# Gorilla-Lab-SCUT/GeoA3

Hardware: AMD Instinct MI355X
Metric: attack-iterations/sec (B=250, N=1024) (higher is better)
Workload: dtype f32; 1 GPU; configs[1]: PointNet 1024-pt, 250 instances sharded over 1 GPU(s) (250 on rank 0), full GeoA3 (CE + CD 1.0 + HD 0.1 + curvature 1.0 k=16), untargeted; instances_per_gpu=250, global_batch=250, npoint=1024, knn=16, classes=40, wide_mode=f16x2, presteps=150, parallelism=instance-sharded x1

## Files before the change

geoa3_amd/csrc/geom_slab.hip:

```cpp
#include <utility>
#include "geom_internal.h"
#include "geom_knn_self.h"
#include "profile.h"

namespace {

constexpr int SB_T = 1024;
constexpr int SB_NB = 512;
constexpr int SB_PPT = 8;
constexpr int SK_BLOCK = 256;
constexpr int SK_CHUNK = 1024;

struct alignas(128) SlabGeo {
  float lo, inv_w;
  int axis, pad;
};
constexpr int SB_PITCH = 544;

__device__ __forceinline__ int slab_bin(float v, float lo, float inv_w) {
  const int c = (int)floorf((v - lo) * inv_w);
  return c < 0 ? 0 : (c > SB_NB - 1 ? SB_NB - 1 : c);
}

__global__ __launch_bounds__(SB_T) void slab_bin_kernel(const float* __restrict__ pc, int N, float* __restrict__ sorted,
                                                        int32_t* __restrict__ sidx, int32_t* __restrict__ bstart,
                                                        SlabGeo* __restrict__ geo) {
  __shared__ float s_red[16][6];
  __shared__ int s_cnt[SB_NB], s_start[SB_NB + 1], s_wsum[16];
  const int b = blockIdx.x, tid = threadIdx.x, lane = tid & 63, wave = tid >> 6;
  const float* P = pc + (size_t)b * 3 * N;
  float px[SB_PPT], py[SB_PPT], pz[SB_PPT];
  float lo[3] = {S_INF, S_INF, S_INF}, hi[3] = {-S_INF, -S_INF, -S_INF};
#pragma unroll
  for (int p = 0; p < SB_PPT; ++p) {
    const int i = tid + p * SB_T;
    if (i < N) {
      px[p] = P[i];
      py[p] = P[N + i];
      pz[p] = P[2 * N + i];
      lo[0] = fminf(lo[0], px[p]); hi[0] = fmaxf(hi[0], px[p]);
      lo[1] = fminf(lo[1], py[p]); hi[1] = fmaxf(hi[1], py[p]);
      lo[2] = fminf(lo[2], pz[p]); hi[2] = fmaxf(hi[2], pz[p]);
    }
  }
#pragma unroll
  for (int c = 0; c < 3; ++c) {
    lo[c] = -wave_max(-lo[c]);
    hi[c] = wave_max(hi[c]);
  }
  if (lane == 0) {
#pragma unroll
    for (int c = 0; c < 3; ++c) {
      s_red[wave][c] = lo[c];
      s_red[wave][3 + c] = hi[c];
    }
  }
  if (tid < SB_NB) s_cnt[tid] = 0;
  __syncthreads();
#pragma unroll
  for (int w = 0; w < 16; ++w)
#pragma unroll
    for (int c = 0; c < 3; ++c) {
      lo[c] = fminf(lo[c], s_red[w][c]);
      hi[c] = fmaxf(hi[c], s_red[w][3 + c]);
    }
  const float ex = hi[0] - lo[0], ey = hi[1] - lo[1], ez = hi[2] - lo[2];
  const int axis = (ex >= ey && ex >= ez) ? 0 : (ey >= ez ? 1 : 2);
  const float alo = axis == 0 ? lo[0] : (axis == 1 ? lo[1] : lo[2]);
  const float ext = axis == 0 ? ex : (axis == 1 ? ey : ez);
  const float inv_w = ext > 1e-30f ? (float)SB_NB / (ext * 1.00001f) : 0.f;
  int bin[SB_PPT];
#pragma unroll
  for (int p = 0; p < SB_PPT; ++p) {
    const int i = tid + p * SB_T;
    if (i < N) {
      bin[p] = slab_bin(axis == 0 ? px[p] : (axis == 1 ? py[p] : pz[p]), alo, inv_w);
      atomicAdd(&s_cnt[bin[p]], 1);
    }
  }
  __syncthreads();
  int c = tid < SB_NB ? s_cnt[tid] : 0, incl = c;
#pragma unroll
  for (int o = 1; o < 64; o <<= 1) {
    const int v = __shfl_up(incl, o, 64);
    if (lane >= o) incl += v;
  }
  if (lane == 63) s_wsum[wave] = incl;
  __syncthreads();
  int base = 0;
#pragma unroll
  for (int w = 0; w < 16; ++w) base += (w < wave) ? s_wsum[w] : 0;
  if (tid < SB_NB) {
    s_start[tid] = base + incl - c;
    s_cnt[tid] = 0;
  }
  if (tid == SB_NB - 1) s_start[SB_NB] = base + incl;
  __syncthreads();
  float* S = sorted + (size_t)b * 3 * N;
#pragma unroll
  for (int p = 0; p < SB_PPT; ++p) {
    const int i = tid + p * SB_T;
    if (i < N) {
      const int pos = s_start[bin[p]] + atomicAdd(&s_cnt[bin[p]], 1);
      S[pos] = px[p];
      S[N + pos] = py[p];
      S[2 * N + pos] = pz[p];
      sidx[(size_t)b * N + pos] = i;
    }
  }
  for (int e = tid; e <= SB_NB; e += SB_T) bstart[(size_t)b * SB_PITCH + e] = s_start[e];
  if (tid == 0) geo[b] = SlabGeo{alo, inv_w, axis, 0};
}

typedef float slab_f2 __attribute__((ext_vector_type(2)));
__device__ __forceinline__ void slab_sqdist2(float nqx, float nqy, float nqz, float x0, float x1, float y0, float y1,
                                             float z0, float z1, float& d0, float& d1) {
#pragma clang fp contract(off)
  const slab_f2 dx = slab_f2{x0, x1} + slab_f2{nqx, nqx};
  const slab_f2 dy = slab_f2{y0, y1} + slab_f2{nqy, nqy};
  const slab_f2 dz = slab_f2{z0, z1} + slab_f2{nqz, nqz};
  const slab_f2 xx = dx * dx, yy = dy * dy, zz = dz * dz;
  const slab_f2 s = xx + yy;
  const slab_f2 d = s + zz;
  d0 = d.x;
  d1 = d.y;
}
__device__ __forceinline__ void slab_negq(float qx, float qy, float qz, float& nqx, float& nqy, float& nqz) {
  nqx = -qx;
  nqy = -qy;
  nqz = -qz;
  asm volatile("" : "+v"(nqx), "+v"(nqy), "+v"(nqz));
}

__device__ __forceinline__ bool slab_lex_less(float da, int ia, float db, int ib) {
  return (da < db) || (da == db && ia < ib);
}

template <int CAP>
__device__ __forceinline__ float slab_compact(uint16_t* cand, float* candd, int cnt, int K, int tid) {
  float kth = S_INF;
  if constexpr (CAP <= 40) {
    unsigned long long key[CAP];
    int rank[CAP];
#pragma unroll
    for (int s = 0; s < CAP; ++s) {
      const unsigned d = __float_as_uint(candd[s * SK_BLOCK + tid]);
      const unsigned i = cand[s * SK_BLOCK + tid];
      key[s] = s < cnt ? ((unsigned long long)d << 32) | i : ~0ull;
      rank[s] = CAP - 1 - s;
    }
#pragma unroll
    for (int i = 0; i < CAP; ++i)
#pragma unroll
      for (int j = i + 1; j < CAP; ++j) {
        unsigned long long m;
        asm volatile("v_cmp_lt_u64 %2, %3, %4\n\tv_subbrev_co_u32 %0, vcc, 0, %0, %2\n\t"
                     "v_addc_co_u32 %1, vcc, 0, %1, %2"
                     : "+v"(rank[i]), "+v"(rank[j]), "=&s"(m)
                     : "v"(key[i]), "v"(key[j])
                     : "vcc");
      }
#pragma unroll
    for (int s = 0; s < CAP; ++s) {
      if (rank[s] < K) {
        const float d = __uint_as_float((unsigned)(key[s] >> 32));
        candd[rank[s] * SK_BLOCK + tid] = d;
        cand[rank[s] * SK_BLOCK + tid] = (uint16_t)key[s];
        if (rank[s] == K - 1) kth = d;
      }
    }
    return kth;
  }
  for (int p = 0; p < K; ++p) {
    float bd = candd[p * SK_BLOCK + tid];
    int bidx = cand[p * SK_BLOCK + tid];
    int bs = p;
    for (int s = p + 1; s < cnt; ++s) {
      const float d = candd[s * SK_BLOCK + tid];
      const int i = cand[s * SK_BLOCK + tid];
      if (slab_lex_less(d, i, bd, bidx)) {
        bd = d;
        bidx = i;
        bs = s;
      }
    }
    if (bs != p) {
      candd[bs * SK_BLOCK + tid] = candd[p * SK_BLOCK + tid];
      cand[bs * SK_BLOCK + tid] = cand[p * SK_BLOCK + tid];
      candd[p * SK_BLOCK + tid] = bd;
      cand[p * SK_BLOCK + tid] = (uint16_t)bidx;
    }
    kth = bd;
  }
  return kth;
}

template <int CAP>
__global__ __launch_bounds__(SK_BLOCK) void knn_slab_kernel(const float* __restrict__ R, int N, int K,
                                                            const int32_t* __restrict__ prior,
                                                            const float* __restrict__ sorted,
                                                            const int32_t* __restrict__ sidx,
                                                            const int32_t* __restrict__ bstart,
                                                            const SlabGeo* __restrict__ geo, float* __restrict__ dists,
                                                            int32_t* __restrict__ idx) {
  extern __shared__ __attribute__((aligned(16))) unsigned char smem[];
  float* s_ref = reinterpret_cast<float*>(smem);
  float* s_cd = s_ref + 3 * SK_CHUNK;
  uint16_t* s_ci = reinterpret_cast<uint16_t*>(s_cd + (size_t)CAP * SK_BLOCK);
  uint16_t* s_id = s_ci + (size_t)CAP * SK_BLOCK;
  __shared__ int s_lo, s_hi;
  const int b = blockIdx.y, tid = threadIdx.x;
  const int pos = blockIdx.x * SK_BLOCK + tid;
  const bool live = pos < N;
  const float* Rb = R + (size_t)b * 3 * N;
  const float* Sb = sorted + (size_t)b * 3 * N;
  const int32_t* Ib = sidx + (size_t)b * N;
  const int32_t* bs = bstart + (size_t)b * SB_PITCH;
  const SlabGeo g = geo[b];
  const int pc = live ? pos : N - 1;
  const float qx = Sb[pc], qy = Sb[N + pc], qz = Sb[2 * N + pc];
  float nqx, nqy, nqz;
  slab_negq(qx, qy, qz, nqx, nqy, nqz);
  const int qo = Ib[pc];
  if (tid == 0) {
    s_lo = SB_NB;
    s_hi = -1;
  }
  float tau = S_INF;
  if (prior != nullptr && live) {
    const int32_t* pr = prior + ((size_t)b * N + qo) * K;
    float t = 0.f;
    bool ok = true;
    for (int m0 = 0; m0 < K; m0 += 8) {
      int j[8];
#pragma unroll
      for (int u = 0; u < 8; ++u) j[u] = m0 + u < K ? pr[m0 + u] : 0;
      float px[8], py[8], pz[8];
#pragma unroll
      for (int u = 0; u < 8; ++u) {
        ok = ok && j[u] >= 0 && j[u] < N;
        const int jc = j[u] < 0 ? 0 : (j[u] >= N ? N - 1 : j[u]);
        px[u] = Rb[jc];
        py[u] = Rb[N + jc];
        pz[u] = Rb[2 * N + jc];
      }
#pragma unroll
      for (int u = 0; u < 8; ++u)
        if (m0 + u < K) t = fmaxf(t, geoa3_sqdist(qx, qy, qz, px[u], py[u], pz[u]));
    }
    if (ok) tau = t;
  }
  if (!live) tau = -1.f;
  __syncthreads();
  if (live) {
    int blo = 0, bhi = SB_NB - 1;
    if (tau < S_INF) {
      const float qa = g.axis == 0 ? qx : (g.axis == 1 ? qy : qz);
      const float r = sqrtf(tau) * 1.00001f + 1e-30f;
      blo = slab_bin(qa - r, g.lo, g.inv_w);
      bhi = slab_bin(qa + r, g.lo, g.inv_w);
    }
    atomicMin(&s_lo, blo);
    atomicMax(&s_hi, bhi);
  }
  __syncthreads();
  int c_lo = bs[s_lo], c_hi = bs[s_hi + 1];

  static_assert(SK_BLOCK == 256, "aoff >> 10 is the count");
  unsigned char* const cdb = reinterpret_cast<unsigned char*>(s_cd);
  unsigned char* const cib = reinterpret_cast<unsigned char*>(s_ci);
  unsigned aoff = 4u * tid;
  int cnt = 0;
  for (int pass = 0; pass < 2; ++pass) {
    for (int c0 = c_lo; c0 < c_hi; c0 += SK_CHUNK) {
      const int cn = min(SK_CHUNK, c_hi - c0);
      const int cn4 = (cn + 3) & ~3;
      __syncthreads();
      for (int j = tid; j < cn4; j += SK_BLOCK) {
        const bool ok = j < cn;
        s_ref[j] = ok ? Sb[c0 + j] : __builtin_nanf("");
        s_ref[SK_CHUNK + j] = ok ? Sb[N + c0 + j] : __builtin_nanf("");
        s_ref[2 * SK_CHUNK + j] = ok ? Sb[2 * N + c0 + j] : __builtin_nanf("");
        s_id[j] = ok ? (uint16_t)Ib[c0 + j] : (uint16_t)0;
      }
      __syncthreads();
      float4 nx = *reinterpret_cast<const float4*>(&s_ref[0]);
      float4 ny = *reinterpret_cast<const float4*>(&s_ref[SK_CHUNK]);
      float4 nz = *reinterpret_cast<const float4*>(&s_ref[2 * SK_CHUNK]);
      for (int j = 0; j < cn4; j += 4) {
        const float4 rx = nx, ry = ny, rz = nz;
        const int jn = j + 4 < SK_CHUNK ? j + 4 : j;
        nx = *reinterpret_cast<const float4*>(&s_ref[jn]);
        ny = *reinterpret_cast<const float4*>(&s_ref[SK_CHUNK + jn]);
        nz = *reinterpret_cast<const float4*>(&s_ref[2 * SK_CHUNK + jn]);
        float da[4];
        slab_sqdist2(nqx, nqy, nqz, rx.x, rx.y, ry.x, ry.y, rz.x, rz.y, da[0], da[1]);
        slab_sqdist2(nqx, nqy, nqz, rx.z, rx.w, ry.z, ry.w, rz.z, rz.w, da[2], da[3]);
        const uint2 ids = *reinterpret_cast<const uint2*>(&s_id[j]);
        const unsigned id4[4] = {ids.x & 0xffffu, ids.x >> 16, ids.y & 0xffffu, ids.y >> 16};
#pragma unroll
        for (int u = 0; u < 4; ++u) {
          *reinterpret_cast<float*>(cdb + aoff) = da[u];
          *reinterpret_cast<uint16_t*>(cib + (aoff >> 1)) = (uint16_t)id4[u];
          aoff += da[u] <= tau ? 4u * SK_BLOCK : 0u;
        }
        if (__builtin_expect(__any(aoff > (unsigned)(CAP - 4) * 4u * SK_BLOCK + 4u * SK_BLOCK - 1u), 0)) {
          cnt = (int)(aoff >> 10);
          if (cnt >= K) {
            tau = slab_compact<CAP>(s_ci, s_cd, cnt, K, tid);
            aoff = (unsigned)K * 4u * SK_BLOCK + 4u * tid;
          }
        }
      }
    }
    cnt = (int)(aoff >> 10);
    const bool short_list = live && cnt < K && K <= N;
    if (!__syncthreads_or(short_list)) break;
    tau = live ? S_INF : -1.f;
    cnt = 0;
    aoff = 4u * tid;
    c_lo = 0;
    c_hi = N;
  }

  if (live) {
    const int keep = cnt < K ? cnt : K;
    slab_compact<CAP>(s_ci, s_cd, cnt, keep, tid);
    float* od = dists + ((size_t)b * N + qo) * K;
    int32_t* oi = idx + ((size_t)b * N + qo) * K;
    for (int m = 0; m < K; ++m) {
      od[m] = m < keep ? s_cd[m * SK_BLOCK + tid] : S_INF;
      oi[m] = m < keep ? (int32_t)s_ci[m * SK_BLOCK + tid] : -1;
    }
  }
}

template <typename F, int... S>
__device__ __forceinline__ void sp_static_for_impl(F&& f, std::integer_sequence<int, S...>) {
  (f(std::integral_constant<int, S>{}), ...);
}
template <int N_, typename F>
__device__ __forceinline__ void sp_static_for(F&& f) {
  sp_static_for_impl(f, std::make_integer_sequence<int, N_>{});
}
__device__ __forceinline__ void sp_count_less(int& r, unsigned long long kj, unsigned long long ki) {
  asm volatile("v_cmp_lt_u64 vcc, %1, %2\n\tv_addc_co_u32 %0, vcc, 0, %0, vcc" : "+v"(r) : "v"(kj), "v"(ki) : "vcc");
}

template <int SP_CAP, bool MULTI>
__global__ __launch_bounds__(SK_BLOCK) __attribute__((amdgpu_waves_per_eu(MULTI ? 3 : 4, MULTI ? 3 : 4))) void knn_slabp_kernel(const float* __restrict__ R, int N, int K,
                                                             const int32_t* __restrict__ prior,
                                                             const float* __restrict__ sorted,
                                                             const int32_t* __restrict__ sidx,
                                                             const int32_t* __restrict__ bstart,
                                                             const SlabGeo* __restrict__ geo, float* __restrict__ dists,
                                                             int32_t* __restrict__ idx) {
  __shared__ __attribute__((aligned(16))) float s_ref[3 * SK_CHUNK];
  __shared__ __attribute__((aligned(16))) uint16_t s_id[SK_CHUNK];
  constexpr int SP_KMAX = 20;
  constexpr int SP_SEED = 3 * SK_CHUNK * 4 + SK_BLOCK * SP_KMAX * 2;
  constexpr int SP_UNION = !MULTI && SP_SEED > SP_CAP * SK_BLOCK * 2 ? SP_SEED : SP_CAP * SK_BLOCK * 2;
  __shared__ __attribute__((aligned(16))) unsigned char s_un[SP_UNION];
  uint16_t* const s_pos = reinterpret_cast<uint16_t*>(s_un);
  __shared__ int s_lo, s_hi;
  const int b = blockIdx.y, tid = threadIdx.x;
  const int pos = blockIdx.x * SK_BLOCK + tid;
  const bool live = pos < N;
  const float* Rb = R + (size_t)b * 3 * N;
  const float* Sb = sorted + (size_t)b * 3 * N;
  const int32_t* Ib = sidx + (size_t)b * N;
  const int32_t* bs = bstart + (size_t)b * SB_PITCH;
  const SlabGeo g = geo[b];
  const int pc = live ? pos : N - 1;
  const float qx = Sb[pc], qy = Sb[N + pc], qz = Sb[2 * N + pc];
  float nqx, nqy, nqz;
  slab_negq(qx, qy, qz, nqx, nqy, nqz);
  const int qo = Ib[pc];
  if (tid == 0) {
    s_lo = SB_NB;
    s_hi = -1;
  }
  float tau = S_INF;
  if (!MULTI && prior != nullptr) {
    float* const s_org = reinterpret_cast<float*>(s_un);
    uint16_t* const s_pri = reinterpret_cast<uint16_t*>(s_un + 3 * SK_CHUNK * 4);
    for (int j = tid; j < 3 * N; j += SK_BLOCK) s_org[j] = Rb[j];
    s_id[tid] = (uint16_t)qo;
    __syncthreads();
    const int w0 = tid & ~63, lane = tid & 63;
    const float inv_k = 1.0f / (float)K;
    for (int e = lane; e < 64 * K; e += 64) {
      const int row = (int)(((float)e + 0.5f) * inv_k), m = e - row * K;
      const int32_t v = prior[((size_t)b * N + s_id[w0 + row]) * K + m];
      s_pri[w0 * K + e] = (uint16_t)(v < 0 || v >= N ? 0xffff : v);
    }
    __syncthreads();
    if (live) {
      float t = 0.f;
      bool ok = true;
      for (int m = 0; m < K; ++m) {
        const unsigned j = s_pri[tid * K + m];
        ok = ok && j != 0xffffu;
        const int jc = j >= (unsigned)N ? N - 1 : (int)j;
        t = fmaxf(t, geoa3_sqdist(qx, qy, qz, s_org[jc], s_org[N + jc], s_org[2 * N + jc]));
      }
      if (ok) tau = t;
    }
  }
  if (MULTI && prior != nullptr && live) {
    const int32_t* pr = prior + ((size_t)b * N + qo) * K;
    float t = 0.f;
    bool ok = true;
    for (int m0 = 0; m0 < K; m0 += 8) {
      int j[8];
#pragma unroll
      for (int u = 0; u < 8; ++u) j[u] = m0 + u < K ? pr[m0 + u] : 0;
      float px[8], py[8], pz[8];
#pragma unroll
      for (int u = 0; u < 8; ++u) {
        ok = ok && j[u] >= 0 && j[u] < N;
        const int jc = j[u] < 0 ? 0 : (j[u] >= N ? N - 1 : j[u]);
        px[u] = Rb[jc];
        py[u] = Rb[N + jc];
        pz[u] = Rb[2 * N + jc];
      }
#pragma unroll
      for (int u = 0; u < 8; ++u)
        if (m0 + u < K) t = fmaxf(t, geoa3_sqdist(qx, qy, qz, px[u], py[u], pz[u]));
    }
    if (ok) tau = t;
  }
  if (!live) tau = -1.f;
  __syncthreads();
  int blo = SB_NB, bhi = -1;
  if (live) {
    blo = 0;
    bhi = SB_NB - 1;
    if (tau < S_INF) {
      const float qa = g.axis == 0 ? qx : (g.axis == 1 ? qy : qz);
      const float r = sqrtf(tau) * 1.00001f + 1e-30f;
      blo = slab_bin(qa - r, g.lo, g.inv_w);
      bhi = slab_bin(qa + r, g.lo, g.inv_w);
    }
    atomicMin(&s_lo, blo);
    atomicMax(&s_hi, bhi);
  }
  const int w_blo = -(int)wave_max(-(float)blo), w_bhi = (int)wave_max((float)bhi);
  int wv_lo = w_blo <= w_bhi ? bs[w_blo] : 0, wv_hi = w_blo <= w_bhi ? bs[w_bhi + 1] : 0;
  __syncthreads();
  int c_lo = bs[s_lo], c_hi = bs[s_hi + 1];

  static_assert(SK_BLOCK == 256, "poff >> 9 is the count");
  unsigned char* const pb = reinterpret_cast<unsigned char*>(s_pos);
  unsigned poff = 2u * tid;
  unsigned long long key[SP_CAP];
  auto load_keys = [&](auto C_, int cnt) {
    sp_static_for<decltype(C_)::value>([&](auto S_) {
      constexpr int s = decltype(S_)::value;
      unsigned p = s_pos[s * SK_BLOCK + tid];
      float d;
      unsigned id;
      if (MULTI) {
        p = p < (unsigned)N ? p : 0u;
        d = geoa3_sqdist(qx, qy, qz, Sb[p], Sb[N + p], Sb[2 * N + p]);
        id = (unsigned)Ib[p];
      } else {
        p &= SK_CHUNK - 1;
        d = geoa3_sqdist(qx, qy, qz, s_ref[p], s_ref[SK_CHUNK + p], s_ref[2 * SK_CHUNK + p]);
        id = s_id[p];
      }
      key[s] = s < cnt ? ((unsigned long long)__float_as_uint(d) << 32) | (id << 16) | p : ~0ull;
      if ((s & 7) == 7) __builtin_amdgcn_sched_barrier(0);
    });
  };
  auto rank_of = [&](auto C_, auto S_) {
    constexpr int s = decltype(S_)::value;
    int r = 0;
    sp_static_for<decltype(C_)::value>([&](auto J_) {
      constexpr int j = decltype(J_)::value;
      if constexpr (j != s) sp_count_less(r, key[j], key[s]);
    });
    return r;
  };
  for (int pass = 0; pass < 2; ++pass) {
   for (int c0 = c_lo; c0 < c_hi; c0 += SK_CHUNK) {
    const int cn = min(SK_CHUNK, c_hi - c0);
    const int cn4 = (cn + 3) & ~3;
    __syncthreads();
    for (int j = tid; j < cn4; j += SK_BLOCK) {
      const bool ok = j < cn;
      s_ref[j] = ok ? Sb[c0 + j] : __builtin_nanf("");
      s_ref[SK_CHUNK + j] = ok ? Sb[N + c0 + j] : __builtin_nanf("");
      s_ref[2 * SK_CHUNK + j] = ok ? Sb[2 * N + c0 + j] : __builtin_nanf("");
      s_id[j] = ok ? (uint16_t)Ib[c0 + j] : (uint16_t)0;
    }
    __syncthreads();
    const int j_lo = min(max(wv_lo - c0, 0), SK_CHUNK - 4) & ~3, j_hi = (min(wv_hi - c0, cn) + 3) & ~3;
    float4 nx = *reinterpret_cast<const float4*>(&s_ref[j_lo]);
    float4 ny = *reinterpret_cast<const float4*>(&s_ref[SK_CHUNK + j_lo]);
    float4 nz = *reinterpret_cast<const float4*>(&s_ref[2 * SK_CHUNK + j_lo]);
    for (int j = j_lo; j < j_hi; j += 4) {
      const float4 rx = nx, ry = ny, rz = nz;
      const int jn = j + 4 < SK_CHUNK ? j + 4 : j;
      nx = *reinterpret_cast<const float4*>(&s_ref[jn]);
      ny = *reinterpret_cast<const float4*>(&s_ref[SK_CHUNK + jn]);
      nz = *reinterpret_cast<const float4*>(&s_ref[2 * SK_CHUNK + jn]);
      float da[4];
      slab_sqdist2(nqx, nqy, nqz, rx.x, rx.y, ry.x, ry.y, rz.x, rz.y, da[0], da[1]);
      slab_sqdist2(nqx, nqy, nqz, rx.z, rx.w, ry.z, ry.w, rz.z, rz.w, da[2], da[3]);
#pragma unroll
      for (int u = 0; u < 4; ++u) {
        *reinterpret_cast<uint16_t*>(pb + poff) = (uint16_t)((MULTI ? c0 : 0) + j + u);
        poff += da[u] <= tau ? 2u * SK_BLOCK : 0u;
      }
      if (__builtin_expect(__any(poff > (unsigned)(SP_CAP - 4) * 2u * SK_BLOCK + 2u * SK_BLOCK - 1u), 0)) {
        const int cnt = (int)(poff >> 9);
        if (cnt >= K) {
          load_keys(std::integral_constant<int, SP_CAP>{}, cnt);
          sp_static_for<SP_CAP>([&](auto S_) {
            constexpr int s = decltype(S_)::value;
            const int r = rank_of(std::integral_constant<int, SP_CAP>{}, S_);
            if (r < K) s_pos[r * SK_BLOCK + tid] = (uint16_t)key[s];
            if (r == K - 1) tau = __uint_as_float((unsigned)(key[s] >> 32));
          });
          poff = (unsigned)K * 2u * SK_BLOCK + 2u * tid;
        }
      }
    }
   }
    const int cnt = (int)(poff >> 9);
    const bool short_list = live && cnt < K && K <= N;
    if (!__syncthreads_or(short_list)) break;
    tau = live ? S_INF : -1.f;
    poff = 2u * tid;
    c_lo = 0;
    c_hi = N;
    wv_lo = 0;
    wv_hi = N;
  }

  if constexpr (MULTI) {
    if (live) {
      const int cnt = (int)(poff >> 9);
      const int keep = cnt < K ? cnt : K;
      constexpr std::integral_constant<int, SP_CAP> C_{};
      load_keys(C_, cnt);
      float* od = dists + ((size_t)b * N + qo) * K;
      int32_t* oi = idx + ((size_t)b * N + qo) * K;
      sp_static_for<SP_CAP>([&](auto S_) {
        constexpr int s = decltype(S_)::value;
        const int r = rank_of(C_, S_);
        if (r < keep) {
          od[r] = __uint_as_float((unsigned)(key[s] >> 32));
          oi[r] = (int32_t)((key[s] >> 16) & 0xffffu);
        }
      });
      for (int m = keep; m < K; ++m) {
        od[m] = S_INF;
        oi[m] = -1;
      }
    }
  } else {
    const int cnt = live ? (int)(poff >> 9) : 0;
    const int keep = cnt < K ? cnt : K;
    const int cls = !__any(cnt > 20) ? 0 : (!__any(cnt > 28) ? 1 : 2);
    constexpr std::integral_constant<int, 20> C20{};
    constexpr std::integral_constant<int, 28> C28{};
    constexpr std::integral_constant<int, SP_CAP> CXX{};
    if (cls == 0) load_keys(C20, cnt);
    else if (cls == 1) load_keys(C28, cnt);
    else load_keys(CXX, cnt);
    __syncthreads();
    float* const s_od = reinterpret_cast<float*>(s_un);
    uint16_t* const s_oi = reinterpret_cast<uint16_t*>(s_ref);
    s_id[tid] = (uint16_t)qo;
    for (int m = keep; m < K; ++m) {
      s_od[tid * K + m] = S_INF;
      s_oi[tid * K + m] = 0xffff;
    }
    auto rank_out = [&](auto C_) {
      sp_static_for<decltype(C_)::value>([&](auto S_) {
        constexpr int s = decltype(S_)::value;
        const int r = rank_of(C_, S_);
        if (r < keep) {
          s_od[tid * K + r] = __uint_as_float((unsigned)(key[s] >> 32));
          s_oi[tid * K + r] = (uint16_t)(key[s] >> 16);
        }
      });
    };
    if (cls == 0) rank_out(C20);
    else if (cls == 1) rank_out(C28);
    else rank_out(CXX);
    __syncthreads();
    const float inv_k = 1.0f / (float)K;
    const int rows = min(SK_BLOCK, N - (int)blockIdx.x * SK_BLOCK);
    for (int e = tid; e < rows * K; e += SK_BLOCK) {
      const int row = (int)(((float)e + 0.5f) * inv_k), m = e - row * K;
      const size_t o = ((size_t)b * N + s_id[row]) * K + m;
      const unsigned v = s_oi[e];
      dists[o] = s_od[e];
      idx[o] = v == 0xffffu ? -1 : (int32_t)v;
    }
  }
}

enum KnnRoute {
  ALLPAIRS = GEOA3_KNN_ROUTE_ALLPAIRS,
  CELLGRID = GEOA3_KNN_ROUTE_CELLGRID,
  SLAB40 = GEOA3_KNN_ROUTE_SLAB40,
  SLAB72 = GEOA3_KNN_ROUTE_SLAB72,
  SLAB96 = GEOA3_KNN_ROUTE_SLAB96,
  SLABP32 = GEOA3_KNN_ROUTE_SLABP32,
  SLABP56 = GEOA3_KNN_ROUTE_SLABP56,
};
constexpr int KNN_SORT_MAX_N = SB_T * SB_PPT;
constexpr int KNN_SHORT_K = 20;
constexpr int KNN_MID_K = 40;
constexpr int KNN_GRID_MIN_N = 2048;
constexpr size_t KNN_DENSE_MIN_WGS = 512;
static_assert(KNN_SORT_MAX_N <= 65535, "positions and original indices travel as 16 bits");

bool knn_self_sizes_ok(int B, int N, int K) { return B > 0 && N > 0 && K > 0 && K <= GEOA3_KNN_MAX_K; }

KnnRoute knn_self_route(int B, int N, int K, int method, bool has_prior, bool scratch_ok) {
  if (!has_prior || !scratch_ok || N > KNN_SORT_MAX_N || K > N) return ALLPAIRS;
  if (method == GEOA3_KNN_SELF_GRID || (method == GEOA3_KNN_SELF_AUTO && (K > KNN_SHORT_K || N >= KNN_GRID_MIN_N)))
    return CELLGRID;
  const size_t wgs = (size_t)((N + SK_BLOCK - 1) / SK_BLOCK) * B;
  const bool positions =
      method != GEOA3_KNN_SELF_SLAB_LISTS && (wgs > KNN_DENSE_MIN_WGS || method == GEOA3_KNN_SELF_SLAB_POSITIONS);
  if (K <= KNN_SHORT_K && N <= SK_CHUNK && positions) return SLABP32;
  if (K <= KNN_MID_K && positions) return SLABP56;
  return K <= KNN_SHORT_K ? SLAB40 : (K <= KNN_MID_K ? SLAB72 : SLAB96);
}

template <int CAP, class Launch>
void launch_slab(Launch&& launch) {
  const size_t lds = 3 * SK_CHUNK * 4 + (size_t)CAP * SK_BLOCK * 6 + SK_CHUNK * 2;
  if (lds > 64 * 1024)
    (void)hipFuncSetAttribute(reinterpret_cast<const void*>(knn_slab_kernel<CAP>), hipFuncAttributeMaxDynamicSharedMemorySize,
                              (int)lds);
  launch(knn_slab_kernel<CAP>, lds);
}

}

extern "C" int64_t geoa3_knn_self_scratch_bytes(int B, int N) {
  if (B <= 0 || N <= 0) return -1;
  const size_t a = knn_self_carve(nullptr, B, N, SB_PITCH, sizeof(SlabGeo)).total, g = geoa3_knn_cellgrid_scratch_bytes(B, N);
  return (int64_t)(a > g ? a : g);
}

extern "C" int geoa3_debug_knn_self_route(int B, int N, int K, int method, int has_prior, int scratch_ok) {
  if (!knn_self_sizes_ok(B, N, K)) return GEOA3_EINVAL;
  return knn_self_route(B, N, K, method, has_prior != 0, scratch_ok != 0);
}

extern "C" int geoa3_knn_self(const float* pc, int B, int N, int K, const int32_t* prior, float* dists, int32_t* idx,
                              void* scratch, int method, void* stream) {
  if (!pc || !dists || !idx || !knn_self_sizes_ok(B, N, K)) return GEOA3_EINVAL;
  hipStream_t s = geoa3_stream(stream);
  geoa3_prof_begin(GEOA3_PROF_KNN, s);
  int rc = GEOA3_OK;
  const bool scratch_ok = scratch && ((uintptr_t)scratch & 255) == 0;
  auto slab = [&](auto kernel, size_t lds) {
    const KnnSelfScratch sc = knn_self_carve(scratch, B, N, SB_PITCH, sizeof(SlabGeo));
    SlabGeo* const geo = static_cast<SlabGeo*>(sc.geo);
    hipLaunchKernelGGL(slab_bin_kernel, dim3(B), dim3(SB_T), 0, s, pc, N, sc.sorted, sc.sidx, sc.start, geo);
    hipLaunchKernelGGL(kernel, dim3((N + SK_BLOCK - 1) / SK_BLOCK, B), dim3(SK_BLOCK), lds, s, pc, N, K, prior, sc.sorted,
                       sc.sidx, sc.start, geo, dists, idx);
    if (hipGetLastError() != hipSuccess) rc = GEOA3_ELAUNCH;
  };
  switch (knn_self_route(B, N, K, method, prior != nullptr, scratch_ok)) {
    case ALLPAIRS: rc = geoa3_launch_knn(pc, pc, B, N, N, K, prior, dists, idx, nullptr, s); break;
    case CELLGRID: rc = geoa3_launch_knn_cellgrid(pc, B, N, K, prior, dists, idx, scratch, s); break;
    case SLAB40: launch_slab<40>(slab); break;
    case SLAB72: launch_slab<72>(slab); break;
    case SLAB96: launch_slab<96>(slab); break;
    case SLABP32: slab(knn_slabp_kernel<32, false>, 0); break;
    case SLABP56: slab(knn_slabp_kernel<56, true>, 0); break;
  }
  geoa3_prof_end(GEOA3_PROF_KNN, s);
  return rc;
}
```

Baseline: 651.8 iterations/s of a 250-instance batch.

## Prefetch slab reference chunk into registers and overlap with prior-gather setup

```diff
diff --git a/geoa3_amd/csrc/geom_slab.hip b/geoa3_amd/csrc/geom_slab.hip
--- a/geoa3_amd/csrc/geom_slab.hip
+++ b/geoa3_amd/csrc/geom_slab.hip
@@ -194,6 +194,37 @@
   }
   return kth;
 }
+
+struct SlabRun {
+  static constexpr int T = SK_CHUNK / SK_BLOCK;
+  float x[T], y[T], z[T];
+  int32_t id[T];
+  __device__ __forceinline__ void request(const float* __restrict__ Sb, const int32_t* __restrict__ Ib, int N, int c0, int cn,
+                                          int tid) {
+#pragma unroll
+    for (int u = 0; u < T; ++u) {
+      const int j = c0 + max(min(tid + u * SK_BLOCK, cn - 1), 0);
+      x[u] = Sb[j];
+      y[u] = Sb[N + j];
+      z[u] = Sb[2 * N + j];
+      id[u] = Ib[j];
+    }
+  }
+  __device__ __forceinline__ void commit(float* s_ref, uint16_t* s_id, int cn, int tid) const {
+    const int cn4 = (cn + 3) & ~3;
+#pragma unroll
+    for (int u = 0; u < T; ++u) {
+      const int j = tid + u * SK_BLOCK;
+      if (j < cn4) {
+        const bool ok = j < cn;
+        s_ref[j] = ok ? x[u] : __builtin_nanf("");
+        s_ref[SK_CHUNK + j] = ok ? y[u] : __builtin_nanf("");
+        s_ref[2 * SK_CHUNK + j] = ok ? z[u] : __builtin_nanf("");
+        s_id[j] = ok ? (uint16_t)id[u] : (uint16_t)0;
+      }
+    }
+  }
+};
 
 template <int CAP>
 __global__ __launch_bounds__(SK_BLOCK) void knn_slab_kernel(const float* __restrict__ R, int N, int K,
@@ -275,14 +306,10 @@
     for (int c0 = c_lo; c0 < c_hi; c0 += SK_CHUNK) {
       const int cn = min(SK_CHUNK, c_hi - c0);
       const int cn4 = (cn + 3) & ~3;
+      SlabRun run;
+      run.request(Sb, Ib, N, c0, cn, tid);
       __syncthreads();
-      for (int j = tid; j < cn4; j += SK_BLOCK) {
-        const bool ok = j < cn;
-        s_ref[j] = ok ? Sb[c0 + j] : __builtin_nanf("");
-        s_ref[SK_CHUNK + j] = ok ? Sb[N + c0 + j] : __builtin_nanf("");
-        s_ref[2 * SK_CHUNK + j] = ok ? Sb[2 * N + c0 + j] : __builtin_nanf("");
-        s_id[j] = ok ? (uint16_t)Ib[c0 + j] : (uint16_t)0;
-      }
+      run.commit(s_ref, s_id, cn, tid);
       __syncthreads();
       float4 nx = *reinterpret_cast<const float4*>(&s_ref[0]);
       float4 ny = *reinterpret_cast<const float4*>(&s_ref[SK_CHUNK]);
@@ -346,6 +373,23 @@
 __device__ __forceinline__ void sp_count_less(int& r, unsigned long long kj, unsigned long long ki) {
   asm volatile("v_cmp_lt_u64 vcc, %1, %2\n\tv_addc_co_u32 %0, vcc, 0, %0, vcc" : "+v"(r) : "v"(kj), "v"(ki) : "vcc");
 }
+
+#ifdef GEOA3_SP_STAMPS
+__device__ unsigned long long g_sp_stamps[8 * 16];
+#define SP_STAMP(i)                                                                                                    \
+  do {                                                                                                                 \
+    if (!MULTI && tid == 0 && blockIdx.x == 1 && (blockIdx.y & 31) == 7 && blockIdx.y < 256)                           \
+      g_sp_stamps[(blockIdx.y >> 5) * 16 + (i)] = __builtin_amdgcn_s_memtime();                                        \
+  } while (0)
+#define SP_STAMP_AFTER(i, v)                                                                                           \
+  do {                                                                                                                 \
+    asm volatile("" ::"v"(v));                                                                                         \
+    SP_STAMP(i);                                                                                                       \
+  } while (0)
+#else
+#define SP_STAMP(i)
+#define SP_STAMP_AFTER(i, v)
+#endif
 
 template <int SP_CAP, bool MULTI>
 __global__ __launch_bounds__(SK_BLOCK) __attribute__((amdgpu_waves_per_eu(MULTI ? 3 : 4, MULTI ? 3 : 4))) void knn_slabp_kernel(const float* __restrict__ R, int N, int K,
@@ -372,11 +416,13 @@
   const int32_t* bs = bstart + (size_t)b * SB_PITCH;
   const SlabGeo g = geo[b];
   const int pc = live ? pos : N - 1;
+  const int qo = Ib[pc];
   const float qx = Sb[pc], qy = Sb[N + pc], qz = Sb[2 * N + pc];
-  float nqx, nqy, nqz;
-  slab_negq(qx, qy, qz, nqx, nqy, nqz);
-  const int qo = Ib[pc];
-  if (tid == 0) {
+  SP_STAMP(0);
+  constexpr bool EARLY = !MULTI;
+  SlabRun run;
+  if (EARLY && prior == nullptr) run.request(Sb, Ib, N, 0, N, tid);
+  if (!EARLY && tid == 0) {
     s_lo = SB_NB;
     s_hi = -1;
   }
@@ -384,16 +430,33 @@
   if (!MULTI && prior != nullptr) {
     float* const s_org = reinterpret_cast<float*>(s_un);
     uint16_t* const s_pri = reinterpret_cast<uint16_t*>(s_un + 3 * SK_CHUNK * 4);
-    for (int j = tid; j < 3 * N; j += SK_BLOCK) s_org[j] = Rb[j];
-    s_id[tid] = (uint16_t)qo;
-    __syncthreads();
+    constexpr int CT = 3 * SK_CHUNK / SK_BLOCK;
+    const int n3 = 3 * N;
+    float cl[CT];
+#pragma unroll
+    for (int u = 0; u < CT; ++u) cl[u] = Rb[min(tid + u * SK_BLOCK, n3 - 1)];
     const int w0 = tid & ~63, lane = tid & 63;
     const float inv_k = 1.0f / (float)K;
-    for (int e = lane; e < 64 * K; e += 64) {
+    int32_t pv[SP_KMAX];
+    SP_STAMP_AFTER(1, qo);
+#pragma unroll
+    for (int u = 0; u < SP_KMAX; ++u) {
+      const int e = min(lane + 64 * u, 64 * K - 1);
       const int row = (int)(((float)e + 0.5f) * inv_k), m = e - row * K;
-      const int32_t v = prior[((size_t)b * N + s_id[w0 + row]) * K + m];
-      s_pri[w0 * K + e] = (uint16_t)(v < 0 || v >= N ? 0xffff : v);
-    }
+      pv[u] = prior[((size_t)b * N + __shfl(qo, row, 64)) * K + m];
+    }
+    if constexpr (EARLY) run.request(Sb, Ib, N, 0, N, tid);
+#pragma unroll
+    for (int u = 0; u < CT; ++u) s_org[tid + u * SK_BLOCK] = cl[u];
+    SP_STAMP(2);
+#pragma unroll
+    for (int u = 0; u < SP_KMAX; ++u) asm volatile("" : "+v"(pv[u]));
+#pragma unroll
+    for (int u = 0; u < SP_KMAX; ++u) {
+      const int e = lane + 64 * u;
+      if (e < 64 * K) s_pri[w0 * K + e] = (uint16_t)(pv[u] < 0 || pv[u] >= N ? 0xffff : pv[u]);
+    }
+    SP_STAMP(3);
     __syncthreads();
     if (live) {
       float t = 0.f;
@@ -431,7 +494,10 @@
     if (ok) tau = t;
   }
   if (!live) tau = -1.f;
-  __syncthreads();
+  SP_STAMP(4);
+  float nqx, nqy, nqz;
+  slab_negq(qx, qy, qz, nqx, nqy, nqz);
+  if (!EARLY) __syncthreads();
   int blo = SB_NB, bhi = -1;
   if (live) {
     blo = 0;
@@ -442,13 +508,22 @@
       blo = slab_bin(qa - r, g.lo, g.inv_w);
       bhi = slab_bin(qa + r, g.lo, g.inv_w);
     }
-    atomicMin(&s_lo, blo);
-    atomicMax(&s_hi, bhi);
+    if (!EARLY) {
+      atomicMin(&s_lo, blo);
+      atomicMax(&s_hi, bhi);
+    }
   }
   const int w_blo = -(int)wave_max(-(float)blo), w_bhi = (int)wave_max((float)bhi);
   int wv_lo = w_blo <= w_bhi ? bs[w_blo] : 0, wv_hi = w_blo <= w_bhi ? bs[w_bhi + 1] : 0;
+  if constexpr (EARLY) run.commit(s_ref, s_id, N, tid);
+  SP_STAMP(5);
   __syncthreads();
-  int c_lo = bs[s_lo], c_hi = bs[s_hi + 1];
+  int c_lo = 0, c_hi = N;
+  if constexpr (!EARLY) {
+    c_lo = bs[s_lo];
+    c_hi = bs[s_hi + 1];
+  }
+  SP_STAMP_AFTER(6, wv_lo + wv_hi + c_lo + c_hi);
 
   static_assert(SK_BLOCK == 256, "poff >> 9 is the count");
   unsigned char* const pb = reinterpret_cast<unsigned char*>(s_pos);
@@ -485,16 +560,12 @@
   for (int pass = 0; pass < 2; ++pass) {
    for (int c0 = c_lo; c0 < c_hi; c0 += SK_CHUNK) {
     const int cn = min(SK_CHUNK, c_hi - c0);
-    const int cn4 = (cn + 3) & ~3;
-    __syncthreads();
-    for (int j = tid; j < cn4; j += SK_BLOCK) {
-      const bool ok = j < cn;
-      s_ref[j] = ok ? Sb[c0 + j] : __builtin_nanf("");
-      s_ref[SK_CHUNK + j] = ok ? Sb[N + c0 + j] : __builtin_nanf("");
-      s_ref[2 * SK_CHUNK + j] = ok ? Sb[2 * N + c0 + j] : __builtin_nanf("");
-      s_id[j] = ok ? (uint16_t)Ib[c0 + j] : (uint16_t)0;
-    }
-    __syncthreads();
+    if constexpr (!EARLY) {
+      run.request(Sb, Ib, N, c0, cn, tid);
+      __syncthreads();
+      run.commit(s_ref, s_id, cn, tid);
+      __syncthreads();
+    }
     const int j_lo = min(max(wv_lo - c0, 0), SK_CHUNK - 4) & ~3, j_hi = (min(wv_hi - c0, cn) + 3) & ~3;
     float4 nx = *reinterpret_cast<const float4*>(&s_ref[j_lo]);
     float4 ny = *reinterpret_cast<const float4*>(&s_ref[SK_CHUNK + j_lo]);
@@ -538,6 +609,7 @@
     wv_lo = 0;
     wv_hi = N;
   }
+  SP_STAMP(7);
 
   if constexpr (MULTI) {
     if (live) {
@@ -591,6 +663,7 @@
     if (cls == 0) rank_out(C20);
     else if (cls == 1) rank_out(C28);
     else rank_out(CXX);
+    SP_STAMP(8);
     __syncthreads();
     const float inv_k = 1.0f / (float)K;
     const int rows = min(SK_BLOCK, N - (int)blockIdx.x * SK_BLOCK);
@@ -601,6 +674,7 @@
       dists[o] = s_od[e];
       idx[o] = v == 0xffffu ? -1 : (int32_t)v;
     }
+    SP_STAMP(9);
   }
 }
 
@@ -650,6 +724,12 @@
   const size_t a = knn_self_carve(nullptr, B, N, SB_PITCH, sizeof(SlabGeo)).total, g = geoa3_knn_cellgrid_scratch_bytes(B, N);
   return (int64_t)(a > g ? a : g);
 }
+
+#ifdef GEOA3_SP_STAMPS
+extern "C" int geoa3_debug_sp_stamps(unsigned long long* out) {
+  return hipMemcpyFromSymbol(out, HIP_SYMBOL(g_sp_stamps), sizeof(g_sp_stamps)) == hipSuccess ? 0 : -1;
+}
+#endif
 
 extern "C" int geoa3_debug_knn_self_route(int B, int N, int K, int method, int has_prior, int scratch_ok) {
   if (!knn_self_sizes_ok(B, N, K)) return GEOA3_EINVAL;
```

Result: faster. 659.2 iterations/s of a 250-instance batch (median of 6 runs) (+1.1%).
